# NREL/SSRS

Hardware: AMD Instinct MI355X
Metric: simulated tracks/sec (whole node) (higher is better)
Workload: dtype f64

## Files before the change

ssrs_amd/csrc/tracks.hip:

```cpp
#include <rocrand/rocrand_philox4x32_10.h>
#include <hipcub/hipcub.hpp>

#include <cmath>
#include <cstdlib>
#include <cstring>
#include <new>
#include <vector>

#include "common.h"
#include "track_plan.h"
#include "track_policy.h"

namespace ssrs {

__host__ __device__ constexpr int dr_of(int k) { return k / 3 - 1; }
__host__ __device__ constexpr int dc_of(int k) { return k % 3 - 1; }
#define SSRS_NINV_DIAG 0.70710677f

constexpr uint32_t restriction(int d)
{
    const int dr = dr_of(d), dc = dc_of(d);
    uint32_t m = 0;
    for (int k = 0; k < 9; ++k) {
        bool ok = false;
        if (dr == 0 && dc == 0) ok = true;
        else if (dr != 0 && dc != 0)
            ok = (dr_of(k) == dr || dr_of(k) == 0) && (dc_of(k) == dc || dc_of(k) == 0);
        else if (dr == 0) ok = dc_of(k) == dc;
        else ok = dr_of(k) == dr;
        if (ok && k != 4) m |= 1u << k;
    }
    return m;
}
constexpr uint64_t pack_restrictions(int first, int count)
{
    uint64_t v = 0;
    for (int i = 0; i < count; ++i) v |= static_cast<uint64_t>(restriction(first + i)) << (9 * i);
    return v;
}
constexpr uint64_t kRestrictLo = pack_restrictions(0, 7);
constexpr uint64_t kRestrictHi = pack_restrictions(7, 2);
constexpr uint32_t kAllButCentre = restriction(4);
static_assert(restriction(0) == 0b000001011u, "(-1,-1) -> k in {0,1,3}");
static_assert(restriction(7) == 0b111000000u, "(1,0) -> k in {6,7,8}");
static_assert(kAllButCentre == 0b111101111u, "(0,0) -> all but centre");

__device__ __forceinline__ uint32_t restriction_of(uint32_t d)
{
    const uint64_t v = d < 7 ? (kRestrictLo >> (9 * d)) : (kRestrictHi >> (9 * (d - 7)));
    return static_cast<uint32_t>(v) & 0x1FFu;
}

constexpr uint32_t candidates(int d)
{
    uint32_t v = 0;
    int n = 0;
    for (int k = 0; k < 9 && n < 3; ++k)
        if ((restriction(d) >> k) & 1u) v |= static_cast<uint32_t>(k < 4 ? k : k - 1) << (3 * n++);
    return v;
}
constexpr uint64_t pack_candidates(int first, int count)
{
    uint64_t v = 0;
    for (int i = 0; i < count; ++i) v |= static_cast<uint64_t>(candidates(first + i)) << (9 * i);
    return v;
}
constexpr uint64_t kCandLo = pack_candidates(0, 7), kCandHi = pack_candidates(7, 2);
static_assert(candidates(7) == (5u | (6u << 3) | (7u << 6)), "(1,0) -> table slots 5,6,7");
static_assert(candidates(5) == (2u | (4u << 3) | (7u << 6)), "(0,1) -> k = 2,5,8 = slots 2,4,7");

__device__ __forceinline__ uint32_t candidates_of(uint32_t d)
{
    const uint64_t v = d < 7 ? (kCandLo >> (9 * d)) : (kCandHi >> (9 * (d - 7)));
    return static_cast<uint32_t>(v) & 0x1FFu;
}

constexpr int kRingK[8] = {7, 8, 5, 2, 1, 0, 3, 6};
constexpr int ring_of_k(int k)
{
    for (int c = 0; c < 8; ++c)
        if (kRingK[c] == k) return c;
    return 8;
}
constexpr bool ring_matches_restrictions()
{
    for (int c = 0; c < 8; ++c) {
        const uint32_t m = (1u << kRingK[(c + 7) % 8]) | (1u << kRingK[c]) | (1u << kRingK[(c + 1) % 8]);
        if (m != restriction(kRingK[c])) return false;
    }
// ... 478 lines not shown
template <typename KeyT>
__global__ __launch_bounds__(kBlock) void k_plan_keys(const int32_t *__restrict__ start_rc,
                                                     long long ntracks, PlanGeom g,
                                                     KeyT *__restrict__ keys,
                                                     int32_t *__restrict__ vals, TrackCtl *ctl, int par_bits)
{
    const long long t = blockIdx.x * static_cast<long long>(kBlock) + threadIdx.x;
    int par = 0x7fffffff;
    if (t < ntracks) {
        int perp;
        plan_coords(g, start_rc[2 * t], start_rc[2 * t + 1], par, perp);
        par = par < 0 ? 0 : par;
        perp = perp < 0 ? 0 : perp;
        const int top = (1 << par_bits) - 1;
        keys[t] = (static_cast<KeyT>(perp > top ? top : perp) << par_bits) | static_cast<KeyT>(par > top ? top : par);
        vals[t] = static_cast<int32_t>(t);
    }
    __shared__ int s_min;
    if (threadIdx.x == 0) s_min = 0x7fffffff;
    __syncthreads();
#pragma unroll
    for (int off = 32; off > 0; off >>= 1) {
        const int o = __shfl_down(par, off);
        par = o < par ? o : par;
    }
    if ((threadIdx.x & 63) == 0 && par != 0x7fffffff) atomicMin(&s_min, par);
    __syncthreads();
    if (threadIdx.x == 0 && s_min != 0x7fffffff) atomicMin(&ctl->par_min, static_cast<uint32_t>(s_min));
}

__device__ __forceinline__ int wander_window_of(const WanderWindows *__restrict__ w, int n, int row, int col)
{
    int id = n;
    for (int q = n - 1; q >= 0; --q)
        if (static_cast<uint32_t>(row - w->r0[q]) < static_cast<uint32_t>(kWinRows) &&
            static_cast<uint32_t>(col - w->c0[q]) < static_cast<uint32_t>(kWinCols)) id = q;
    return id;
}

enum { MODE_PRIOR = 0, MODE_UPDRAFT = 1, MODE_FLUIDFLOW = 2, MODE_TABLE = 3 };

struct RoamEntry;

struct StepArgs {
    int rows, cols, burnin, memory;
    long long max_k;
    double nu;
    const double *prior;
    const double *updraft;
    const float *potential;
    const double *table;
    unsigned long long seed, track_base;
    uint32_t *hist;
    int16_t *end_rc;
    int32_t *lengths;
    int16_t *traj;
    const long long *traj_off;
    TrackState *state;
    const int32_t *list_in;
    int32_t *list_out;
    TrackCtl *ctl;
    int launch;
    int fast;
    int steps;
    int coherent;
    uint32_t *visits;
    long long visit_stride;
    uint32_t cap;
    long long it_base;
    int plane_shift;
    uint32_t guard;
    int v16_offset;
    int pf_dir, pf_rc;
    uint32_t vcap;
    const double *thr;
    const uint8_t *zmask;
    uint32_t *hist_copies;
    int ncopies;
    const WanderWindows *wander;
    const RoamEntry *roam;
    const void *fine;
    int roam_stop;
    int cheap_exact;
    unsigned long long *dbg_buf;
    int debug_roam;
    uint32_t vis_r, vis_c;
};

__global__ __launch_bounds__(kBlock) void k_tracks_init(
    const int32_t *__restrict__ start_rc, long long ntracks, int rows, int cols,
    uint32_t *hist, int16_t *traj, const long long *traj_off, int32_t *lengths,
    int16_t *end_rc, TrackState *state, TrackCtl *ctl, PlanGeom g, int coherent, uint32_t cap)
{
    const long long t = blockIdx.x * static_cast<long long>(kBlock) + threadIdx.x;
    if (t < kXcd) {
        const long long left = ntracks - t * static_cast<long long>(cap);
        ctl->count[0][t] = static_cast<uint32_t>(left < 0 ? 0 : (left > cap ? cap : left));
        ctl->count[1][t] = ctl->count[2][t] = ctl->count[3][t] = 0;
        if (t == 0) ctl->steps = 0;
    }
    if (t >= ntracks) return;
    const int row = start_rc[2 * t], col = start_rc[2 * t + 1];
    TrackState s;
    s.dirs = 0x44444444u;
    uint32_t delay = 0;
    if (coherent) {
        int par, perp;
        plan_coords(g, row, col, par, perp);
        par = par < 0 ? 0 : par;
        const uint32_t pmin = ctl->par_min;
        delay = static_cast<uint32_t>(par) > pmin ? static_cast<uint32_t>(par) - pmin : 0u;
        if (delay > 0x7FFFFFu) delay = 0x7FFFFFu;
        delay &= ~1u;
    }
    s.aux = kAllButCentre | (delay << 9);
    if (row < 0 || col < 0 || row >= rows || col >= cols) {
        atomicOr(&ctl->error, 1u);
        s.pos = 0;
        s.k = -1;
        if (lengths) lengths[t] = 0;
        if (end_rc) { end_rc[2 * t] = -1; end_rc[2 * t + 1] = -1; }
    } else {
        s.pos = row | (col << 16);
        s.k = 0;
        if (hist) atomicAdd(&hist[static_cast<size_t>(row) * cols + col], 1u);
        if (traj)
            reinterpret_cast<uint32_t *>(traj)[traj_off[t]] =
                static_cast<uint32_t>(row & 0xFFFF) | (static_cast<uint32_t>(col) << 16);
    }
    state[t] = s;
}

template <int MODE>
__global__ __launch_bounds__(kBlock) void k_step_tracks(const StepArgs a)
{
    TrackCtl *ctl = a.ctl;
    const int in_slot = a.launch & 3, out_slot = (a.launch + 1) & 3;
    const uint32_t xcd = blockIdx.x % kXcd;
    const uint32_t nlive = ctl->count[in_slot][xcd];
    const uint32_t il = (blockIdx.x / kXcd) * kBlock + threadIdx.x;
    const uint32_t i = xcd * a.cap + il;
    const uint32_t iv = xcd * a.vcap + il;
    if (blockIdx.x == 0 && threadIdx.x < kXcd)
        ctl->count[(a.launch + 2) & 3][threadIdx.x] = 0;
    if ((il & ~63u) >= nlive) return;

    bool active = il < nlive;
    const int32_t t = active ? (a.list_in ? a.list_in[i] : static_cast<int32_t>(i)) : 0;
    TrackState s = {0, -1, 0, 0};
    if (active) s = a.state[t];
    active = active && s.k >= 0;
    int row = s.pos & 0xFFFF, col = (s.pos >> 16) & 0xFFFF;
    int k = s.k;
    const int max_k = static_cast<int>(a.max_k);
    uint32_t dirs = s.dirs, run = s.aux & 0x1FFu;
    const long long rel64 = (a.coherent ? static_cast<long long>(s.aux >> 9) : 0) -
                            static_cast<long long>(a.launch) * a.steps;
    const int release = rel64 > 0x7fffffffLL ? 0x7fffffff : (rel64 < 0 ? 0 : static_cast<int>(rel64));
    const unsigned long long track = a.track_base + static_cast<unsigned long long>(t);
    const long long toff = (a.traj && active) ? a.traj_off[t] : 0;
    const long long troom = (a.traj && active) ? a.traj_off[t + 1] - toff : 0;
    uint32_t pend_a = 0, pend_b = 0;
    bool have_pending = false;
    uint32_t moved = 0;
    int last_it = -1;

// ... 1072 lines not shown
struct FineEntry { uint32_t t1, t2; };
struct FinePrior { uint32_t zero_t1[8], zero_t2[8], reversal; };

__host__ __device__ __forceinline__ uint32_t fine_fixed(double x)
{
    const double v = x * 4294967296.0 + 0.5;
    return v >= 4294967295.0 ? 0xFFFFFFFFu : static_cast<uint32_t>(static_cast<unsigned long long>(v));
}

template <bool HAS_POT>
__global__ __launch_bounds__(kBlock) void k_fine_build(const double *__restrict__ updraft, const float *__restrict__ potential,
                                                      FineEntry *__restrict__ out, int rows, int cols, int tiles_x, int ntiles,
                                                      const FinePrior fp)
{
    constexpr int LW = kTabW + 2, LH = kTabH + 2;
    __shared__ double s_inv[LW * LH];
    __shared__ float s_pot[LW * LH];
    const int t = xcd_band(blockIdx.x, ntiles);
    const int r0 = (t / tiles_x) * kTabH, c0 = (t % tiles_x) * kTabW;
    for (int i = threadIdx.x; i < LW * LH; i += kBlock) {
        const int lr = i / LW, lc = i - lr * LW;
        int gr = r0 - 1 + lr, gc = c0 - 1 + lc;
        gr = gr < 0 ? 0 : (gr >= rows ? rows - 1 : gr);
        gc = gc < 0 ? 0 : (gc >= cols ? cols - 1 : gc);
        const size_t g = static_cast<size_t>(gr) * cols + gc;
        const double v = updraft[g];
        const double w = v != v ? v : (v > 1e-06 ? v : 1e-06);
        s_inv[i] = 1.0 / w;
        s_pot[i] = HAS_POT ? potential[g] : 0.f;
    }
    __syncthreads();
    const int lc = static_cast<int>(threadIdx.x % kTabW) + 1;
    const int col = c0 + lc - 1;
    if (col >= cols) return;
    for (int lr = static_cast<int>(threadIdx.x / kTabW) + 1; lr <= kTabH; lr += kBlock / kTabW) {
        const int row = r0 + lr - 1;
        if (row >= rows) break;
        const size_t cell = static_cast<size_t>(row) * cols + col;
        const bool interior = row > 0 && col > 0 && row < rows - 1 && col < cols - 1;
        double w[9];
        bool bad = !interior;
        if (interior) {
            const double ic = s_inv[lr * LW + lc];
            const float pc = s_pot[lr * LW + lc];
#pragma unroll
            for (int j = 0; j < 9; ++j) {
                const int o = (lr + dr_of(j)) * LW + lc + dc_of(j);
                w[j] = 2.0 / (ic + s_inv[o]);
                if (HAS_POT) {
                    const float d = pc - s_pot[o];
                    const float ninv = (j == 4) ? 0.f : ((j & 1) ? 1.f : SSRS_NINV_DIAG);
                    const float e = d * ninv;
                    w[j] = w[j] * static_cast<double>(e);
                }
                bad |= !(w[j] - w[j] == 0.0);
                w[j] = w[j] > 0.0 ? w[j] : 0.0;
            }
        }
        FineEntry en[8];
#pragma unroll
        for (int rc = 0; rc < 8; ++rc) {
            const uint32_t ord = ring_order(rc);
            const int ring3[3] = {(rc + 7) % 8, rc, (rc + 1) % 8};
            const int ka = kRingK[ring3[ord & 3u]], kb = kRingK[ring3[(ord >> 2) & 3u]], kc = kRingK[ring3[(ord >> 4) & 3u]];
            FineEntry e = {0xFFFFFFFFu, 0u};
            if (!bad) {
                const double ab = w[ka] + w[kb], tot = ab + w[kc];
                if (tot == 0.0) {
                    if (!((fp.reversal >> rc) & 1u)) { e.t1 = fp.zero_t1[rc]; e.t2 = fp.zero_t2[rc]; }
                } else if (tot - tot == 0.0) {
                    e.t1 = fine_fixed(w[ka] / tot);
                    e.t2 = fine_fixed(ab / tot);
                    if (e.t1 > e.t2) e.t1 = e.t2;
                }
            }
            en[rc] = e;
        }
        uint4 *dst = reinterpret_cast<uint4 *>(out + cell * 8);
#pragma unroll
        for (int q = 0; q < 4; ++q) dst[q] = make_uint4(en[2 * q].t1, en[2 * q].t2, en[2 * q + 1].t1, en[2 * q + 1].t2);
    }
}

template <bool REV, int BT = kBlock>
__global__ __launch_bounds__(BT) void k_step_roam(const StepArgs a, const ThrPrior pr)
{
    __shared__ uint32_t s_win[kWinRows * kWinCols];
    __shared__ int s_box[4];
    __shared__ int s_wid[BT / 64];
    for (int q = threadIdx.x; q < kWinRows * kWinCols; q += BT) s_win[q] = 0u;
    if (threadIdx.x == 0) { s_box[0] = s_box[1] = 0x7fffffff; s_box[2] = s_box[3] = -1; }
    __syncthreads();
    TrackCtl *ctl = a.ctl;
    const int in_slot = a.launch & 3, out_slot = (a.launch + 1) & 3;
    const uint32_t xcd = blockIdx.x % kXcd;
    const uint32_t nlive = ctl->count[in_slot][xcd];
    const uint32_t il = (blockIdx.x / kXcd) * BT + threadIdx.x;
    const uint32_t i = xcd * a.cap + il;
    if (blockIdx.x == 0 && threadIdx.x < kXcd) ctl->count[(a.launch + 2) & 3][threadIdx.x] = 0;

    bool live0 = il < nlive;
    int32_t t = live0 ? (a.list_in ? a.list_in[i] : static_cast<int32_t>(i)) : 0;
    if (t < 0) { live0 = false; t = 0; }
    TrackState s = {0, -1, 0, 0};
    if (live0) s = a.state[t];
    uint32_t rc = static_cast<uint32_t>(kRingOfK >> (4 * (s.dirs & 0xFu))) & 0xFu;
    live0 = live0 && s.k >= 0 && rc < 8u;
    rc &= 7u;
    int row = s.pos & 0xFFFF, col = (s.pos >> 16) & 0xFFFF;
    int win_r0 = 0, win_c0 = 0;
    {
        int r_lo = live0 ? row : 0x7fffffff, r_hi = live0 ? row : -1, c_lo = live0 ? col : 0x7fffffff, c_hi = live0 ? col : -1;
#pragma unroll
        for (int off = 32; off > 0; off >>= 1) {
            int o = __shfl_xor(r_lo, off); r_lo = o < r_lo ? o : r_lo;
            o = __shfl_xor(r_hi, off); r_hi = o > r_hi ? o : r_hi;
            o = __shfl_xor(c_lo, off); c_lo = o < c_lo ? o : c_lo;
            o = __shfl_xor(c_hi, off); c_hi = o > c_hi ? o : c_hi;
        }
        if ((threadIdx.x & 63) == 0 && r_hi >= 0) {
            atomicMin(&s_box[0], r_lo); atomicMin(&s_box[1], c_lo);
            atomicMax(&s_box[2], r_hi); atomicMax(&s_box[3], c_hi);
        }
        __syncthreads();
        const bool fits = s_box[2] - s_box[0] < kWinRows && s_box[3] - s_box[1] < kWinCols;
        const int nwin = a.wander->n;
        int wid = live0 && nwin > 0 ? wander_window_of(a.wander, nwin, row, col) : 0x7fffffff;
        wid = wid >= nwin ? 0x7fffffff : wid;
        {
            const unsigned long long lm = __ballot(wid != 0x7fffffff);
            wid = lm ? __shfl(wid, __ffsll(static_cast<long long>(lm)) - 1) : 0x7fffffff;
        }
        if ((threadIdx.x & 63) == 0) s_wid[threadIdx.x >> 6] = wid;
        __syncthreads();
        wid = 0x7fffffff;
        for (int q = BT / 64 - 1; q >= 0; --q) wid = s_wid[q] != 0x7fffffff ? s_wid[q] : wid;
        if (wid != 0x7fffffff && threadIdx.x == 0) {
            s_box[0] = a.wander->r0[wid]; s_box[2] = s_box[0] + kWinRows - 1;
            s_box[1] = a.wander->c0[wid]; s_box[3] = s_box[1] + kWinCols - 1;
        }
        const bool placed = wid != 0x7fffffff;
        __syncthreads();
        if (!placed && !fits && threadIdx.x == 0) { s_box[0] = r_lo; s_box[1] = c_lo; s_box[2] = r_hi; s_box[3] = c_hi; }
        __syncthreads();
        if (s_box[2] >= 0) {
            win_r0 = (s_box[0] + s_box[2] + 1 - kWinRows) / 2;
            win_c0 = (s_box[1] + s_box[3] + 1 - kWinCols) / 2;
        }
    }
    const char *pair = reinterpret_cast<const char *>(a.roam);
    const uint32_t ucols = static_cast<uint32_t>(a.cols);
    const uint32_t last_cell = static_cast<uint32_t>(a.rows) * ucols - 1u;
    int k = s.k;
    const long long rel64 = (a.coherent ? static_cast<long long>(s.aux >> 9) : 0) + 1 - a.it_base;
    const int rel = rel64 > 0x3fffffffLL ? 0x3fffffff : (rel64 < 0 ? 0 : static_cast<int>(rel64));
    const long long left = a.max_k - k;
    uint32_t span = !live0 ? 0u : (left > 0x3fffffffLL ? 0x3fffffffu : (left < 0 ? 0u : static_cast<uint32_t>(left)));
    const int blk0 = (k - rel) >> 1;
    const unsigned long long track = a.track_base + static_cast<unsigned long long>(t);
    const char *tab = reinterpret_cast<const char *>(a.table);
    const uint32_t psh = static_cast<uint32_t>(a.plane_shift);
    const uint32_t rev_e = pr.rev_e;
    uint32_t win_stray = 0, n_fine = 0;
    const void *fine = a.fine;

    int wr = 0, wc = 0, lcell = 0;
// ... 9 lines not shown
    };
    enter(rel == 0);
    const uint32_t rev_rc4 = 4u * pr.rev_rc;

    auto slow_step = [&](const uint32_t w0, const uint32_t w1) __attribute__((always_inline)) {
        const uint32_t ufi = w0 >> 16;
        const uint32_t cell = static_cast<uint32_t>(row) * ucols + static_cast<uint32_t>(col);
        const uint32_t e = *reinterpret_cast<const uint32_t *>(tab + (a.guard + (rc << psh)) + (cell << 2));
        const int32_t d1 = static_cast<int32_t>(ufi) - static_cast<int32_t>(e & 0xFFFFu);
        const int32_t d2 = static_cast<int32_t>(ufi) - static_cast<int32_t>(e >> 16);
        const bool burn = k <= a.burnin;
        bool special = (static_cast<uint32_t>(d1 + 1) < 2u) | (static_cast<uint32_t>(d2 + 1) < 2u) | (d1 < d2);
        if (burn) special |= (row <= 1) | (row >= a.rows - 2) | (col >= a.cols - 2);
        uint32_t nc;
        int br = row, bc = col;
        if (!special) {
            const uint32_t ord = static_cast<uint32_t>(kRingOrder >> (6u * rc)) & 63u;
            const uint32_t neg = (static_cast<uint32_t>(d1) >> 31) + (static_cast<uint32_t>(d2) >> 31);
            nc = (rc + 7u + ((ord >> (4u - 2u * neg)) & 3u)) & 7u;
        } else {
            if (e == kThrBoundary && !burn) { span = 0u; return; }
            bool exact = true;
            nc = 0;
            if (fine && !(d1 < d2) && !(burn && ((row <= 1) | (row >= a.rows - 2) | (col >= a.cols - 2)))) {
                const uint2 f = reinterpret_cast<const uint2 *>(fine)[(cell << 3) | rc];
                const uint32_t u32 = (w0 & ~31u) | (w1 >> 27);
                const long long f1 = static_cast<long long>(u32) - static_cast<long long>(f.x);
                const long long f2 = static_cast<long long>(u32) - static_cast<long long>(f.y);
                const bool unsure = (f.x > f.y) | (static_cast<unsigned long long>(f1 + 1) < 2ull) | (static_cast<unsigned long long>(f2 + 1) < 2ull);
                if (!unsure) {
                    const uint32_t ord = static_cast<uint32_t>(kRingOrder >> (6u * rc)) & 63u;
                    const uint32_t neg = (f1 < 0 ? 1u : 0u) + (f2 < 0 ? 1u : 0u);
                    nc = (rc + 7u + ((ord >> (4u - 2u * neg)) & 3u)) & 7u;
                    exact = false;
                    ++n_fine;
                }
            }
            if (e == kThrReversal && !burn) {
                int idx = 0;
                bool near = false;
#pragma unroll
                for (int q = 0; q < 9; ++q) {
                    const int32_t d = static_cast<int32_t>(ufi) - static_cast<int32_t>(pr.thr9[q]);
                    idx += d >= 0 ? 1 : 0;
                    near |= static_cast<uint32_t>(d + 1) < 2u;
                }
                const uint32_t pnc = static_cast<uint32_t>(kRingOfK >> (4 * (idx > 8 ? 4 : idx))) & 0xFu;
                if (!near && pnc < 8u) { nc = pnc; exact = false; }
            }
            if (exact) {
                int er = row, ec = col;
                if (burn) {
                    if (er <= 1) er += 2; else if (er >= a.rows - 2) er -= 2;
                    if (ec <= 0) ec += 2; else if (ec >= a.cols - 2) ec -= 2;
                }
                double w[9];
                if (a.potential) window_weights<true>(a.updraft, a.potential, a.cols, er, ec, w);
                else window_weights<false>(a.updraft, a.potential, a.cols, er, ec, w);
                double prr[9];
#pragma unroll
                for (int j = 0; j < 9; ++j) prr[j] = a.prior[j];
                const uint32_t last = static_cast<uint32_t>(kKOfRing >> (4 * rc)) & 0xFu;
                const int idx = choose_move(w, prr, 1.0, restriction_of(last), words_to_uniform(w0, w1), true);
                nc = static_cast<uint32_t>(kRingOfK >> (4 * idx)) & 0xFu;
                br = er; bc = ec;
            }
        }
        row = br + static_cast<int>((kRingDr >> (2u * nc)) & 3u) - 1;
        col = bc + static_cast<int>((kRingDc >> (2u * nc)) & 3u) - 1;
        rc = nc;
        ++k;
        const uint32_t hr = static_cast<uint32_t>(row - win_r0), hc = static_cast<uint32_t>(col - win_c0);
        if (hr < static_cast<uint32_t>(kWinRows) && hc < static_cast<uint32_t>(kWinCols)) {
            atomicAdd(&s_win[hr * kWinCols + hc], 1u);
        } else {
            atomicAdd(&a.hist[static_cast<uint32_t>(row) * ucols + static_cast<uint32_t>(col)], 1u);
            ++win_stray;
        }
    };

    int it = 0;
    uint32_t n_pairs = 0, n_slow = 0;
    const unsigned long long t_begin = a.debug_roam ? __builtin_amdgcn_s_memtime() : 0ull;
    auto one_pair = [&]() __attribute__((always_inline)) {
        const uint4 w4 = philox_block_b3(a.seed, track, static_cast<unsigned long long>(static_cast<uint32_t>(blk0 + (it >> 1))));
        const uint32_t ufa = w4.x >> 16, ufb = w4.z >> 16;
        const bool st_a = static_cast<uint32_t>(it - rel) < span, st_b = static_cast<uint32_t>(it + 1 - rel) < span;
        const uint32_t q0 = E.x, qa = E.y, qb = E.z, qc = E.w;
        const uint32_t rc0 = rc;
        const uint32_t rc04 = 4u * rc0;
        const bool rva = REV && q0 == kThrReversal;
        const uint32_t eua = rva ? rev_e : q0;
        const uint32_t t4a = rva ? rev_rc4 : rc04;
        const bool ga1 = ufa >= (eua & 0xFFFFu), ga2 = ufa >= (eua >> 16);
        const uint32_t nxa = ga2 ? kRingNext2 : (ga1 ? kRingNext1 : kRingNext0);
        const uint32_t nca = (nxa >> t4a) & 7u, nca4 = 4u * nca;
        const uint32_t q1 = ga2 ? qc : (ga1 ? qb : qa);
        const int dra = __builtin_amdgcn_sbfe(static_cast<int>(kRingDrS), nca4, 2u), dca = __builtin_amdgcn_sbfe(static_cast<int>(kRingDcS), nca4, 2u);
        const int cell_a = lcell + __mul24(dra, a.cols) + dca;
        const bool rvb = REV && q1 == kThrReversal;
        const uint32_t eub = rvb ? rev_e : q1;
        const uint32_t t4b = rvb ? rev_rc4 : nca4;
        const bool gb1 = ufb >= (eub & 0xFFFFu), gb2 = ufb >= (eub >> 16);
        const uint32_t nxb = gb2 ? kRingNext2 : (gb1 ? kRingNext1 : kRingNext0);
        const uint32_t ncb = (nxb >> t4b) & 7u, ncb4 = 4u * ncb;
        const int drb = __builtin_amdgcn_sbfe(static_cast<int>(kRingDrS), ncb4, 2u), dcb = __builtin_amdgcn_sbfe(static_cast<int>(kRingDcS), ncb4, 2u);
        const int cell_b = cell_a + __mul24(drb, a.cols) + dcb;
        {
            const uint32_t cb = static_cast<uint32_t>(cell_b) < last_cell ? static_cast<uint32_t>(cell_b) : last_cell;
            E = *reinterpret_cast<const uint4 *>(pair + ((cb << 7) | (ncb4 << 2)));
        }
        const int wra = wr + dra, wca = wc + dca, wrb = wra + drb, wcb = wca + dcb;
        const int32_t a1 = static_cast<int32_t>(ufa) - static_cast<int32_t>(eua & 0xFFFFu);
        const int32_t a2 = static_cast<int32_t>(ufa) - static_cast<int32_t>(eua >> 16);
        const int32_t b1 = static_cast<int32_t>(ufb) - static_cast<int32_t>(eub & 0xFFFFu);
        const int32_t b2 = static_cast<int32_t>(ufb) - static_cast<int32_t>(eub >> 16);
        const bool special = (static_cast<uint32_t>(a1 + 1) < 2u) | (static_cast<uint32_t>(a2 + 1) < 2u) | (a1 < a2) |
                             (static_cast<uint32_t>(b1 + 1) < 2u) | (static_cast<uint32_t>(b2 + 1) < 2u) | (b1 < b2);
        const bool go = fast & st_a & st_b & !special;
        const bool in_a = go & (static_cast<uint32_t>(wra) < static_cast<uint32_t>(kWinRows)) & (static_cast<uint32_t>(wca) < static_cast<uint32_t>(kWinCols));
        const bool in_b = go & (static_cast<uint32_t>(wrb) < static_cast<uint32_t>(kWinRows)) & (static_cast<uint32_t>(wcb) < static_cast<uint32_t>(kWinCols));
        const bool out = go & !(in_a & in_b);
        const bool slow = (st_a | st_b) & !go;
        const unsigned long long rare = __ballot(out | slow);
        atomicAdd(&s_win[in_a ? (wra << 8) + wca : 0], in_a ? 1u : 0u);
        atomicAdd(&s_win[in_b ? (wrb << 8) + wcb : 0], in_b ? 1u : 0u);
        k += go ? 2 : 0;
        wr = go ? wrb : wr;
        wc = go ? wcb : wc;
        lcell = go ? cell_b : lcell;
        rc = go ? ncb : rc0;
        ++n_pairs;
        if (__builtin_expect(rare != 0ull, 0)) {
            if (__any(out)) {
#ifdef SSRS_PROBE_NO_STRAY_ATOMICS
                if (go && !in_a) ++win_stray;
                if (go && !in_b) ++win_stray;
#else
                if (go && !in_a) { atomicAdd(&a.hist[cell_a], 1u); ++win_stray; }
                if (go && !in_b) { atomicAdd(&a.hist[cell_b], 1u); ++win_stray; }
#endif
            }
            if (__any(slow)) {
                ++n_slow;
                if (slow) {
                    if (fast) { row = win_r0 + wr; col = win_c0 + wc; }
#pragma unroll 1
                    for (int h = 0; h < 2; ++h)
                        if (static_cast<uint32_t>(it + h - rel) < span) slow_step(h ? w4.z : w4.x, h ? w4.w : w4.y);
                    enter(true);
                }
            }
        }
        it += 2;
    };
    const uint32_t stop_stamp = static_cast<uint32_t>(a.launch) + 1u;
    uint32_t stop_seen = 0u;
    bool stopped = false;
    for (; it + 8 <= a.steps; ) {
        const unsigned long long stepping = __ballot(static_cast<uint32_t>(it - rel) < span), waiting = __ballot(it < rel && span != 0u);
        const bool stop_now = a.roam_stop && waiting == 0ull &&
                              static_cast<uint32_t>(__builtin_amdgcn_readfirstlane(static_cast<int>(stop_seen))) == stop_stamp;
        if (((stepping | waiting) == 0ull) | stop_now) { stopped = stop_now; break; }
        if (a.roam_stop) stop_seen = __hip_atomic_load(&ctl->roam_stop, __ATOMIC_RELAXED, __HIP_MEMORY_SCOPE_AGENT);
#pragma unroll
        for (int u = 0; u < 4; ++u) one_pair();
    }
    for (; it < a.steps && !stopped; ) {
        if (!__any(static_cast<uint32_t>(it - rel) < span || (it < rel && span != 0u))) break;
        one_pair();
    }
    if (a.roam_stop && !stopped && it >= a.steps && (threadIdx.x & 63) == 0) atomicMax(&ctl->roam_stop, stop_stamp);
    if (fast) { row = win_r0 + wr; col = win_c0 + wc; }
    {
        uint32_t nf = n_fine;
#pragma unroll
        for (int off = 32; off > 0; off >>= 1) nf += __shfl_down(nf, off);
        if ((threadIdx.x & 63) == 0 && nf) atomicAdd(&ctl->pad, nf);
    }
    if ((threadIdx.x & 63) == 0 && n_pairs) {
        atomicAdd(&ctl->roam_pairs, static_cast<unsigned long long>(n_pairs));
        if (n_slow) atomicAdd(&ctl->roam_slow, static_cast<unsigned long long>(n_slow));
        if (a.debug_roam) {
            const unsigned long long dt = __builtin_amdgcn_s_memtime() - t_begin;
            atomicAdd(&ctl->dbg_tsum, dt);
            atomicMax(&ctl->dbg_tmax, dt);
            atomicAdd(&ctl->dbg_waves, 1ull);
            atomicMax(&ctl->dbg_slowmax, (static_cast<unsigned long long>(n_slow) << 32) | n_pairs);
        }
    }
#ifdef SSRS_DEBUG_WAVE_DUMP
    if (a.debug_roam && a.launch == SSRS_DEBUG_WAVE_DUMP && a.dbg_buf) {
        const unsigned long long dt = __builtin_amdgcn_s_memtime() - t_begin;
        const int lanes = __popcll(__ballot(live0));
        uint32_t wst = win_stray;
        for (int off = 32; off > 0; off >>= 1) wst += __shfl_down(wst, off);
        if ((threadIdx.x & 63) == 0) {
            unsigned long long *r = a.dbg_buf + 8ull * (blockIdx.x * (BT / 64) + (threadIdx.x >> 6));
            r[0] = dt; r[1] = static_cast<unsigned long long>(lanes); r[2] = n_pairs; r[3] = n_slow; r[4] = wst;
            r[5] = static_cast<unsigned long long>(win_r0); r[6] = static_cast<unsigned long long>(win_c0);
            r[7] = static_cast<uint32_t>(__popcll(__ballot(fast)));
        }
    }
#endif
    __syncthreads();
    for (int q = threadIdx.x; q < kWinRows * kWinCols; q += BT) {
        const uint32_t n = s_win[q];
        if (n) atomicAdd(&a.hist[static_cast<uint32_t>(win_r0 + q / kWinCols) * ucols + static_cast<uint32_t>(win_c0 + q % kWinCols)], n);
    }
    {
        unsigned long long ws = win_stray;
#pragma unroll
        for (int off = 32; off > 0; off >>= 1) ws += __shfl_down(ws, off);
        if ((threadIdx.x & 63) == 0 && ws) atomicAdd(&ctl->strays, ws);
    }
    const bool active = live0 && span != 0u && k < static_cast<int>(a.max_k);
    if (live0 && !active) {
        if (a.lengths) a.lengths[t] = static_cast<int32_t>(k + 1);
        if (a.end_rc) reinterpret_cast<uint32_t *>(a.end_rc)[t] = (static_cast<uint32_t>(row) & 0xFFFFu) | (static_cast<uint32_t>(col) << 16);
    }
    __shared__ uint32_t s_surv[BT / 64 + 1];
    const int lane = threadIdx.x & 63, wv = threadIdx.x >> 6;
    const int nsurv = __popcll(__ballot(active));
    if (lane == 0) s_surv[wv] = static_cast<uint32_t>(nsurv);
    __syncthreads();
    if (threadIdx.x == 0) {
        uint32_t tot = 0;
        for (int q = 0; q < BT / 64; ++q) tot += s_surv[q];
        s_surv[BT / 64] = tot ? atomicAdd(&ctl->count[out_slot][xcd], static_cast<uint32_t>(BT)) : 0xFFFFFFFFu;
    }
    __syncthreads();
    const uint32_t basei = s_surv[BT / 64];
    if (basei != 0xFFFFFFFFu) {
        a.list_out[xcd * a.cap + basei + threadIdx.x] = active ? t : -1;
        if (active) {
            TrackState o;
            o.pos = static_cast<int32_t>((static_cast<uint32_t>(row) & 0xFFFFu) | (static_cast<uint32_t>(col) << 16));
            o.k = k;
            o.dirs = static_cast<uint32_t>(kKOfRing >> (4 * rc)) & 0xFu;
            o.aux = s.aux;
            a.state[t] = o;
        }
    }
    unsigned long long mv = live0 ? static_cast<unsigned long long>(k - s.k) : 0ull;
#pragma unroll
    for (int off = 32; off > 0; off >>= 1) mv += __shfl_down(mv, off);
    if (lane == 0 && mv) atomicAdd(&ctl->steps, mv);
}

constexpr int kBinThreads = 1024;
constexpr int kBinCells = 30720;
__global__ __launch_bounds__(kBinThreads) void k_bin_visits(const uint32_t *__restrict__ visits,
                                                           long long stride,
// ... 871 lines not shown
    return SSRS_OK;
}

extern "C" size_t ssrs_transition_ring_bytes(int rows, int cols)
{
    if (rows <= 0 || cols <= 0) return 0;
    const size_t cells = static_cast<size_t>(rows) * static_cast<size_t>(cols);
    return ring_mask_offset(rows, cols) + (cells + 3) / 4 * 4;
}

extern "C" int ssrs_transition_ring_build(const double *updraft, const float *potential,
                                          float *ring, int rows, int cols, void *stream)
{
    SSRS_REQUIRE(updraft && ring, "ssrs_transition_ring_build: updraft/ring is NULL");
    SSRS_REQUIRE(rows >= 3 && cols >= 3, "ssrs_transition_ring_build: need rows, cols >= 3");
    SSRS_REQUIRE((reinterpret_cast<uintptr_t>(ring) & 7u) == 0,
                 "ssrs_transition_ring_build: ring must be 8-byte aligned");
    const int tx = (cols + kTabW - 1) / kTabW, ty = (rows + kTabH - 1) / kTabH, nt = tx * ty;
    hipLaunchKernelGGL(k_transition_table<true>, dim3(static_cast<unsigned>(nt)), dim3(kBlock), 0,
                       as_stream(stream), updraft, potential, static_cast<void *>(ring), rows, cols, tx, nt);
    SSRS_HIP_CHECK(hipGetLastError());
    return SSRS_OK;
}

static size_t thr_guard_bytes(int cols) { return align_up((static_cast<size_t>(cols) + 2) * 4, 256); }

extern "C" size_t ssrs_transition_thr_bytes(int rows, int cols)
{
    if (rows <= 0 || cols <= 0) return 0;
    return (static_cast<size_t>(8) << thr_plane_shift(rows, cols)) + 2 * thr_guard_bytes(cols);
}

extern "C" int ssrs_transition_thr_build(const double *updraft, const float *potential,
                                         const double *prior, float *thr, int rows, int cols, void *stream)
{
    SSRS_REQUIRE(updraft && thr && prior, "ssrs_transition_thr_build: updraft/prior/thr is NULL");
    SSRS_REQUIRE(rows >= 3 && cols >= 3, "ssrs_transition_thr_build: need rows, cols >= 3");
    SSRS_REQUIRE(static_cast<size_t>(rows) * static_cast<size_t>(cols) <= (1ull << 26),
                 "ssrs_transition_thr_build: the table and its guard bands are addressed with 32-bit offsets (rows * cols <= 2^26)");
    SSRS_REQUIRE((reinterpret_cast<uintptr_t>(thr) & 63u) == 0,
                 "ssrs_transition_thr_build: table must be 64-byte aligned");
    ThrPrior pr;
    prior_tables(prior, &pr);
    const int tx = (cols + kTabW - 1) / kTabW, ty = (rows + kTabH - 1) / kTabH, nt = tx * ty;
    uint32_t *planes = reinterpret_cast<uint32_t *>(reinterpret_cast<char *>(thr) + thr_guard_bytes(cols));
    ThrHeader *header = reinterpret_cast<ThrHeader *>(thr);
    PriorArg heading;
    for (int k = 0; k < 9; ++k) heading.v[k] = prior[k];
    if (potential)
        hipLaunchKernelGGL(k_transition_thr<true>, dim3(static_cast<unsigned>(nt)), dim3(kBlock), 0, as_stream(stream),
                           updraft, potential, planes, rows, cols, tx, nt, pr, thr_plane_shift(rows, cols), header, heading);
    else
        hipLaunchKernelGGL(k_transition_thr<false>, dim3(static_cast<unsigned>(nt)), dim3(kBlock), 0, as_stream(stream),
                           updraft, potential, planes, rows, cols, tx, nt, pr, thr_plane_shift(rows, cols), header, heading);
    SSRS_HIP_CHECK(hipGetLastError());
    return SSRS_OK;
}

extern "C" int ssrs_uniform_selftest(uint64_t seed, const uint64_t *track, const uint64_t *step,
                                     double *out, size_t n, void *stream)
{
    SSRS_REQUIRE(track && step && out, "ssrs_uniform_selftest: NULL pointer");
    if (n == 0) return SSRS_OK;
    hipLaunchKernelGGL(k_uniform_selftest, dim3(static_cast<unsigned>((n + 255) / 256)), dim3(256),
                       0, as_stream(stream), seed, track, step, out, n);
    SSRS_HIP_CHECK(hipGetLastError());
    return SSRS_OK;
}


struct TrackCall {
    const SsrsTrackParams *p;
    const double *updraft; const float *potential; const double *table;
    const int32_t *start_rc; int64_t ntracks; uint64_t seed, track_id_base;
    uint32_t *hist; int16_t *end_rc; int32_t *lengths; int16_t *traj; const int64_t *traj_offsets;
    void *workspace; size_t workspace_bytes; void *stream;
    SsrsTrajRecorder *rec;
    unsigned long long *hist64;
};

struct TrackSwitches {
    bool debug, debug_roam;
    bool roam_stop, cheap_exact, block_window, fine_table, roam_table, rev, deal_contiguous, rebalance, grow_steps;
    long long roam_wide_from;
    int roam_width;
    int roam_shuffle;
};

static TrackSwitches read_track_switches()
{
    auto set = [](const char *name) { return std::getenv(name) != nullptr; };
    TrackSwitches sw;
    sw.debug = set("SSRS_TRACKS_DEBUG");
    sw.debug_roam = set("SSRS_TRACKS_DEBUG_ROAM");
    sw.roam_stop = !set("SSRS_TRACKS_NO_ROAM_STOP");
    sw.cheap_exact = !set("SSRS_TRACKS_NO_CHEAP_EXACT");
    sw.block_window = !set("SSRS_TRACKS_NO_BLOCK_WINDOW");
    sw.fine_table = !set("SSRS_TRACKS_NO_FINE_TABLE");
    sw.roam_table = !set("SSRS_TRACKS_NO_ROAM_TABLE");
    sw.rev = !set("SSRS_TRACKS_NO_REV");
    sw.deal_contiguous = !set("SSRS_TRACKS_DEAL_ROUND_ROBIN");
    sw.rebalance = !set("SSRS_TRACKS_NO_REBALANCE");
    sw.grow_steps = !set("SSRS_TRACKS_FIXED_STEPS");
    sw.roam_wide_from = static_cast<long long>(kDealBlocks + kWanderWindows - 2) * kBlock + 1;
    if (const char *e = std::getenv("SSRS_TRACKS_ROAM_WIDE")) sw.roam_wide_from = std::atoll(e);
    sw.roam_width = 0;
    if (const char *e = std::getenv("SSRS_TRACKS_ROAM_WIDTH")) { const int w = std::atoi(e); if (w == 1 || w == 2 || w == 4) sw.roam_width = w; }
    sw.roam_shuffle = 16;
    if (const char *e = std::getenv("SSRS_TRACKS_ROAM_SHUFFLE")) sw.roam_shuffle = std::atoi(e);
    return sw;
}

static_assert(offsetof(TrackCtl, steps) == kSlotSteps * sizeof(uint32_t) &&
              offsetof(TrackCtl, strays) == kSlotSteps * sizeof(uint32_t) + sizeof(unsigned long long), "read-back slot");

struct TrackEvents {
    hipEvent_t first = nullptr, last = nullptr;
    hipEvent_t batch[kRing] = {};
    bool own_batch = false;
    std::vector<hipEvent_t> marks;
    std::vector<int> kind;
    TrackEvents() = default;
    TrackEvents(const TrackEvents &) = delete;
    TrackEvents &operator=(const TrackEvents &) = delete;
    ~TrackEvents()
    {
        for (hipEvent_t e : marks) (void)hipEventDestroy(e);
        if (own_batch)
            for (hipEvent_t e : batch)
                if (e) (void)hipEventDestroy(e);
        if (first) (void)hipEventDestroy(first);
        if (last) (void)hipEventDestroy(last);
    }
};

static int check_track_args(const TrackCall &c)
{
    const SsrsTrackParams *p = c.p;
    SSRS_REQUIRE(p != nullptr, "ssrs_tracks_simulate: params is NULL");
    SSRS_REQUIRE(c.hist64 == nullptr || c.hist != nullptr, "ssrs_tracks_simulate_h64: the 32-bit raster the kernels count into is NULL");
    SSRS_REQUIRE(p->rows >= 5 && p->cols >= 5, "ssrs_tracks_simulate: need rows, cols >= 5 (got %d x %d)",
                 p->rows, p->cols);
    SSRS_REQUIRE(p->rows <= 32767 && p->cols <= 32767,
                 "ssrs_tracks_simulate: rows, cols must fit int16 trajectories (<= 32767)");
    SSRS_REQUIRE(p->memory_parameter >= 0 && p->memory_parameter <= 8,
                 "ssrs_tracks_simulate: memory_parameter must be in 0..8 (got %d)",
                 p->memory_parameter);
    SSRS_REQUIRE(p->max_moves >= 0 && p->max_moves < (1ll << 31) - 1,
                 "ssrs_tracks_simulate: max_moves out of range");
    SSRS_REQUIRE(p->burnin >= 0, "ssrs_tracks_simulate: burnin must be >= 0");
    SSRS_REQUIRE(c.ntracks >= 0 && c.ntracks < (1ll << 31) - 64, "ssrs_tracks_simulate: bad ntracks");
    SSRS_REQUIRE(!(c.potential && !c.updraft && !c.table),
                 "ssrs_tracks_simulate: potential_field needs updraft_field (reference raises)");
    SSRS_REQUIRE(!(c.traj && !c.traj_offsets), "ssrs_tracks_simulate: traj needs traj_offsets");
    SSRS_REQUIRE(!(c.table && (reinterpret_cast<uintptr_t>(c.table) & 63u)),
                 "ssrs_tracks_simulate: table must be 64-byte aligned");
    return SSRS_OK;
}

struct TrackRun {
    const TrackCall c;
    const SsrsTrackParams *p;
    const TrackSwitches sw;
    hipStream_t st;
    Workspace ws = {};
    uint32_t *host_counts = nullptr;
    int S = 0, mode = 0, mode0 = 0;
    bool profile = false, coherent = false, lean = false, ring = false, thr = false;
    PlanGeom geom = {};
    ThrPrior thr_prior = {};
    StepArgs a = {};
    uint32_t ntc = 0, ntiles = 0;
    size_t ncell = 0;
    bool roam_ok = false, rev = false, wander_sort_ok = false, v16_ok = false;
    uint32_t *hist_t = nullptr;
    uint32_t *copies_ptr = nullptr;
    int ncopies = 0;
    bool copies_live = false;
    unsigned long long private_visits = 0;
    bool roam_ready = false;
    int roam_width = 1;
    TrackPolicy pol;
    int launch = 0, batches = 0, last_Sl = 0;
    long long it_done = 0;
    int window_launches = 0, tile_launches = 0, block_window_launches = 0, roam_launches = 0, roam_wide_launches = 0;
    int slot_row[kRing] = {};
// ... 42 lines not shown
    if (bad)
        return set_error(SSRS_ERR_INVALID, "ssrs_tracks_simulate: `table` is not a threshold table built by "
                         "ssrs_transition_thr_build for this %d x %d raster and params->prior (nothing was launched)",
                         p->rows, p->cols);
    return SSRS_OK;
}

int TrackRun::plan_and_init()
{
    const int64_t ntracks = c.ntracks;
    SSRS_HIP_CHECK(hipEventCreate(&ev.first));
    SSRS_HIP_CHECK(hipEventCreate(&ev.last));
    SSRS_HIP_CHECK(hipEventRecord(ev.first, st));
    {
        PriorArg pa;
        for (int k = 0; k < 9; ++k) pa.v[k] = p->prior[k];
        const ThrHeader *header = (p->flags & SSRS_TRACKS_THR_TABLE) ? reinterpret_cast<const ThrHeader *>(c.table) : nullptr;
        hipLaunchKernelGGL(k_ctl_init, dim3(1), dim3(64), 0, st, ws.ctl, pa, ws.thr, ws.wander, header, p->rows, p->cols);
        SSRS_HIP_CHECK(hipGetLastError());
    }
    coherent = (p->flags & SSRS_TRACKS_NO_SCHEDULE) == 0;
    const unsigned blocks = static_cast<unsigned>((ntracks + kBlock - 1) / kBlock);
    if (coherent) {
        double vr = 0.0, vc = 0.0;
        for (int k = 0; k < 9; ++k) { vr += p->prior[k] * dr_of(k); vc += p->prior[k] * dc_of(k); }
        const double nrm = std::sqrt(vr * vr + vc * vc);
        geom.cos_t = nrm > 0.0 ? vr / nrm : 1.0;
        geom.sin_t = nrm > 0.0 ? vc / nrm : 0.0;
        geom.offset = p->rows + p->cols;
        int par_bits = 1;
        while ((1ll << par_bits) <= 2ll * geom.offset) ++par_bits;
        size_t temp_bytes = ws.sort_temp_bytes;
        if (2 * par_bits <= 32) {
            uint32_t *k0 = reinterpret_cast<uint32_t *>(ws.keys[0]), *k1 = reinterpret_cast<uint32_t *>(ws.keys[1]);
            hipLaunchKernelGGL(k_plan_keys<uint32_t>, dim3(blocks), dim3(kBlock), 0, st, c.start_rc,
                               static_cast<long long>(ntracks), geom, k0, ws.list[1], ws.ctl, par_bits);
            SSRS_HIP_CHECK(hipGetLastError());
            SSRS_HIP_CHECK(hipcub::DeviceRadixSort::SortPairs(
                ws.sort_temp, temp_bytes, k0, k1, ws.list[1], ws.list[0], static_cast<int>(ntracks), 0, 2 * par_bits, st));
        } else {
            hipLaunchKernelGGL(k_plan_keys<unsigned long long>, dim3(blocks), dim3(kBlock), 0, st, c.start_rc,
                               static_cast<long long>(ntracks), geom, ws.keys[0], ws.list[1], ws.ctl, par_bits);
            SSRS_HIP_CHECK(hipGetLastError());
            SSRS_HIP_CHECK(hipcub::DeviceRadixSort::SortPairs(
                ws.sort_temp, temp_bytes, ws.keys[0], ws.keys[1], ws.list[1], ws.list[0],
                static_cast<int>(ntracks), 0, 2 * par_bits, st));
        }
    }
    hipLaunchKernelGGL(k_tracks_init, dim3(blocks), dim3(kBlock), 0, st, c.start_rc,
                       static_cast<long long>(ntracks), p->rows, p->cols, c.hist, c.traj,
                       reinterpret_cast<const long long *>(c.traj_offsets), c.lengths, c.end_rc,
                       ws.state, ws.ctl, geom, coherent ? 1 : 0, ws.cap);
    SSRS_HIP_CHECK(hipGetLastError());

    S = p->steps_per_launch > 0 ? p->steps_per_launch : 512;
    profile = (p->flags & SSRS_TRACKS_PROFILE) != 0;
    mode = c.table ? MODE_TABLE : (c.updraft ? (c.potential ? MODE_FLUIDFLOW : MODE_UPDRAFT) : MODE_PRIOR);
    mode0 = c.updraft ? (c.potential ? MODE_FLUIDFLOW : MODE_UPDRAFT) : MODE_PRIOR;
    a.rows = p->rows; a.cols = p->cols; a.burnin = p->burnin; a.memory = p->memory_parameter;
    a.max_k = p->max_moves; a.nu = p->scaling_parameter;
    a.prior = ws.ctl->prior;
    a.updraft = c.updraft; a.potential = c.potential; a.table = c.table;
    a.seed = c.seed; a.track_base = c.track_id_base;
    a.hist = c.hist; a.end_rc = c.end_rc; a.lengths = c.lengths; a.traj = c.traj;
    a.traj_off = reinterpret_cast<const long long *>(c.traj_offsets);
    a.state = ws.state; a.ctl = ws.ctl; a.steps = S;
    a.fast = ((p->flags & SSRS_TRACKS_EXACT_ONLY) == 0 && p->scaling_parameter == 1.0) ? 1 : 0;
    a.coherent = coherent ? 1 : 0;
    a.cap = ws.cap;
    a.thr = ws.thr;
    a.wander = ws.wander;
    a.debug_roam = sw.debug_roam ? 1 : 0;
    a.roam_stop = sw.roam_stop ? 1 : 0;
    a.dbg_buf = nullptr;
#ifdef SSRS_DEBUG_WAVE_DUMP
    {
        static unsigned long long *dump_buf = nullptr;
        if (!dump_buf && a.debug_roam && hipMalloc(&dump_buf, 8ull * 8 * 4096 * (kBlock / 64)) != hipSuccess) dump_buf = nullptr;
        if (dump_buf) (void)hipMemsetAsync(dump_buf, 0, 8ull * 8 * 4096 * (kBlock / 64), st);
        a.dbg_buf = dump_buf;
    }
#endif
    a.cheap_exact = sw.cheap_exact ? 1 : 0;
    a.vcap = ws.cap;
    lean = p->memory_parameter == 1 && c.traj == nullptr;
    ring = (p->flags & SSRS_TRACKS_RING_TABLE) != 0;
    thr = (p->flags & SSRS_TRACKS_THR_TABLE) != 0;
    if (thr) {
        SSRS_REQUIRE(!ring && c.table && c.updraft && lean && a.fast && (S & 1) == 0,
                     "ssrs_tracks_simulate: SSRS_TRACKS_THR_TABLE needs table + updraft, memory_parameter 1, "
                     "scaling_parameter 1, no direct trajectory output, no EXACT_ONLY and an even steps_per_launch");
        SSRS_REQUIRE(static_cast<size_t>(p->rows) * static_cast<size_t>(p->cols) <= (1ull << 26),
                     "ssrs_tracks_simulate: the threshold table needs rows * cols <= 2^26");
        prior_tables(p->prior, &thr_prior);
        a.plane_shift = thr_plane_shift(p->rows, p->cols);
        a.guard = static_cast<uint32_t>(thr_guard_bytes(p->cols));
        a.pf_dir = coherent ? (geom.cos_t > 0.98 ? 1 : (geom.cos_t < -0.98 ? -1 : 0)) : 0;
        a.pf_rc = a.pf_dir < 0 ? 4 : 0;
    }
    if (ring)
        SSRS_REQUIRE(c.table && c.updraft && lean && a.fast && (S & 1) == 0,
                     "ssrs_tracks_simulate: SSRS_TRACKS_RING_TABLE needs table + updraft, memory_parameter 1, "
                     "scaling_parameter 1, no trajectory output, no EXACT_ONLY and an even steps_per_launch");
    return SSRS_OK;
}

int TrackRun::choose_front_path()
{
    const int64_t ntracks = c.ntracks;
    uint32_t *const hist = c.hist;
    const double off_axis = std::fabs(geom.sin_t) < std::fabs(geom.cos_t) ? std::fabs(geom.sin_t) : std::fabs(geom.cos_t);
    ntc = static_cast<uint32_t>((p->cols + kTileCols - 1) / kTileCols);
    ntiles = ntc * static_cast<uint32_t>((p->rows + kTileRows - 1) / kTileRows);
    const bool tiles_ok = hist != nullptr && coherent && S <= kVisitSteps && ntracks >= 8192 && ntiles <= kTilesMax &&
                          static_cast<unsigned long long>(ws.cap) * kXcd * static_cast<unsigned long long>(S) < (1ull << 32) &&
                          (p->flags & SSRS_TRACKS_NO_BINNING) == 0;
    bool tiles_on = tiles_ok && off_axis > 0.17;
    const bool want_transposed = coherent && !tiles_on && std::fabs(geom.sin_t) > std::fabs(geom.cos_t);
    const bool binning = hist != nullptr && coherent && S <= kVisitSteps &&
                         (p->flags & SSRS_TRACKS_NO_BINNING) == 0 &&
                         (want_transposed ? p->rows : p->cols) <= kBinCells;
    a.visits = nullptr;
    a.visit_stride = ws.visit_stride;
    bool binning_on = binning && ntracks >= 8192 && !tiles_on;
    const bool never_scattered = (p->flags & SSRS_TRACKS_NO_SCATTERED) != 0;
    const bool scattered = (p->flags & SSRS_TRACKS_SCATTERED) != 0;
    if (scattered) binning_on = tiles_on = false;
    const bool cache_ok = thr && hist != nullptr && !(c.rec && c.rec->complete) && sw.block_window;
    size_t ws_base = align_up(ssrs_tracks_workspace_bytes(ntracks), 256);
    {
        const size_t pb = thr ? pair_table_bytes(ntracks, p->rows, p->cols) : 0;
        if (pb && c.workspace_bytes >= ws_base + pb) {
            ws.roam = reinterpret_cast<RoamEntry *>(static_cast<char *>(c.workspace) + ws_base);
            if (sw.fine_table)
                a.fine = static_cast<char *>(c.workspace) + ws_base +
                         align_up(static_cast<size_t>(p->rows) * static_cast<size_t>(p->cols) * 8 * sizeof(RoamEntry), 256);
            ws_base += pb;
        }
        a.roam = ws.roam;
    }
    roam_ok = cache_ok && ws.roam != nullptr && sw.roam_table;
    rev = thr_prior.rev_ok != 0 && sw.rev;
    wander_sort_ok = ntracks >= kWanderMinTracks &&
                     static_cast<long long>((p->rows + kBinRows - 1) / kBinRows) * ((p->cols + kBinCols - 1) / kBinCols) <= kWanderBins;
    ncell = static_cast<size_t>(p->rows) * static_cast<size_t>(p->cols);
    if (hist && c.workspace_bytes > ws_base) ncopies = static_cast<int>((c.workspace_bytes - ws_base) / (ncell * sizeof(uint32_t)));
    uint32_t *extra = reinterpret_cast<uint32_t *>(static_cast<char *>(c.workspace) + ws_base);
    if (want_transposed && binning_on) {
        if (ncopies >= 1) { hist_t = extra; extra += ncell; --ncopies; }
        else binning_on = false;
    }
    if (hist_t) SSRS_HIP_CHECK(hipMemsetAsync(hist_t, 0, sizeof(uint32_t) * ncell, st));
    ncopies = ncopies > 64 ? 64 : ncopies;
    copies_ptr = ncopies >= 2 ? extra : nullptr;
    a.hist_copies = nullptr;
    a.ncopies = 1;
    a.zmask = ring ? reinterpret_cast<const uint8_t *>(c.table) + ring_mask_offset(p->rows, p->cols) : nullptr;
    v16_ok = 5ll * p->cols <= kBinCells;
    a.v16_offset = geom.offset;

    pol.thr = thr; pol.tiles_ok = tiles_ok; pol.cache_ok = cache_ok; pol.never_scattered = never_scattered;
    pol.front = a.pf_dir != 0; pol.may_rebalance = sw.rebalance; pol.debug = sw.debug; pol.roam_shuffle = sw.roam_shuffle;
    pol.ntracks = ntracks; pol.crossing = p->rows + p->cols;
    pol.binning_on = binning_on; pol.tiles_on = tiles_on; pol.scattered = scattered;
    pol.cached = cache_ok && scattered;
    pol.want_wander_sort = pol.cached;
// ... 568 lines not shown
```

Before: 74580.

## Add steady-state roam loop specializations with lane-mask predication

The roaming step loop now classifies each 8-step trip. When every stepping lane is fast and stays in span for the whole trip, it runs specialized versions of the pair step that drop the per-step span checks and use a precomputed wave mask, converted to a per-lane flag with inverse_ballot. A masked variant also skips the whole trip body for inactive lanes and guards the shared-memory atomics with branches instead of dummy adds. This adds code size, register pressure and more control flow, and the roam-stop flag is read mid-trip from the first active lane.

```diff
diff --git a/ssrs_amd/csrc/tracks.hip b/ssrs_amd/csrc/tracks.hip
--- a/ssrs_amd/csrc/tracks.hip
+++ b/ssrs_amd/csrc/tracks.hip
@@ -5,6 +5,7 @@
 #include <cstdlib>
 #include <cstring>
 #include <new>
+#include <type_traits>
 #include <vector>
 
 #include "common.h"
@@ -649,6 +650,8 @@
     const void *fine;
     int roam_stop;
     int cheap_exact;
+    int roam_steady;
+    int roam_mask;
     unsigned long long *dbg_buf;
     int debug_roam;
     uint32_t vis_r, vis_c;
@@ -1887,6 +1890,11 @@
     }
 }
 
+__device__ __forceinline__ bool lane_of_mask(unsigned long long mask)
+{
+    return __builtin_amdgcn_inverse_ballot_w64(mask);
+}
+
 template <bool REV, int BT = kBlock>
 __global__ __launch_bounds__(BT) void k_step_roam(const StepArgs a, const ThrPrior pr)
 {
@@ -2062,10 +2070,11 @@
     int it = 0;
     uint32_t n_pairs = 0, n_slow = 0;
     const unsigned long long t_begin = a.debug_roam ? __builtin_amdgcn_s_memtime() : 0ull;
-    auto one_pair = [&]() __attribute__((always_inline)) {
-        const uint4 w4 = philox_block_b3(a.seed, track, static_cast<unsigned long long>(static_cast<uint32_t>(blk0 + (it >> 1))));
+    auto one_pair = [&](auto steady_c, auto mask_c, const int itp, unsigned long long &on) __attribute__((always_inline)) -> bool {
+        constexpr bool STEADY = decltype(steady_c)::value, MASK = decltype(mask_c)::value;
+        const uint4 w4 = philox_block_b3(a.seed, track, static_cast<unsigned long long>(static_cast<uint32_t>(blk0 + (itp >> 1))));
         const uint32_t ufa = w4.x >> 16, ufb = w4.z >> 16;
-        const bool st_a = static_cast<uint32_t>(it - rel) < span, st_b = static_cast<uint32_t>(it + 1 - rel) < span;
+        const bool st_a = STEADY || static_cast<uint32_t>(itp - rel) < span, st_b = STEADY || static_cast<uint32_t>(itp + 1 - rel) < span;
         const uint32_t q0 = E.x, qa = E.y, qb = E.z, qc = E.w;
         const uint32_t rc0 = rc;
         const uint32_t rc04 = 4u * rc0;
@@ -2097,20 +2106,26 @@
         const int32_t b2 = static_cast<int32_t>(ufb) - static_cast<int32_t>(eub >> 16);
         const bool special = (static_cast<uint32_t>(a1 + 1) < 2u) | (static_cast<uint32_t>(a2 + 1) < 2u) | (a1 < a2) |
                              (static_cast<uint32_t>(b1 + 1) < 2u) | (static_cast<uint32_t>(b2 + 1) < 2u) | (b1 < b2);
-        const bool go = fast & st_a & st_b & !special;
+        const bool lane_on = STEADY ? lane_of_mask(on) : false;
+        const bool go = STEADY ? (lane_on & !special) : (fast & st_a & st_b & !special);
         const bool in_a = go & (static_cast<uint32_t>(wra) < static_cast<uint32_t>(kWinRows)) & (static_cast<uint32_t>(wca) < static_cast<uint32_t>(kWinCols));
         const bool in_b = go & (static_cast<uint32_t>(wrb) < static_cast<uint32_t>(kWinRows)) & (static_cast<uint32_t>(wcb) < static_cast<uint32_t>(kWinCols));
         const bool out = go & !(in_a & in_b);
-        const bool slow = (st_a | st_b) & !go;
+        const bool slow = STEADY ? (lane_on & special) : ((st_a | st_b) & !go);
         const unsigned long long rare = __ballot(out | slow);
-        atomicAdd(&s_win[in_a ? (wra << 8) + wca : 0], in_a ? 1u : 0u);
-        atomicAdd(&s_win[in_b ? (wrb << 8) + wcb : 0], in_b ? 1u : 0u);
+        if constexpr (MASK) {
+            if (in_a) atomicAdd(&s_win[(wra << 8) + wca], 1u);
+            if (in_b) atomicAdd(&s_win[(wrb << 8) + wcb], 1u);
+        } else {
+            atomicAdd(&s_win[in_a ? (wra << 8) + wca : 0], in_a ? 1u : 0u);
+            atomicAdd(&s_win[in_b ? (wrb << 8) + wcb : 0], in_b ? 1u : 0u);
+        }
         k += go ? 2 : 0;
         wr = go ? wrb : wr;
         wc = go ? wcb : wc;
         lcell = go ? cell_b : lcell;
         rc = go ? ncb : rc0;
-        ++n_pairs;
+        bool any_slow = false;
         if (__builtin_expect(rare != 0ull, 0)) {
             if (__any(out)) {
 #ifdef SSRS_PROBE_NO_STRAY_ATOMICS
@@ -2122,33 +2137,79 @@
 #endif
             }
             if (__any(slow)) {
-                ++n_slow;
+                any_slow = true;
                 if (slow) {
                     if (fast) { row = win_r0 + wr; col = win_c0 + wc; }
 #pragma unroll 1
                     for (int h = 0; h < 2; ++h)
-                        if (static_cast<uint32_t>(it + h - rel) < span) slow_step(h ? w4.z : w4.x, h ? w4.w : w4.y);
+                        if (static_cast<uint32_t>(itp + h - rel) < span) slow_step(h ? w4.z : w4.x, h ? w4.w : w4.y);
                     enter(true);
                 }
+                if constexpr (STEADY) on &= __ballot(fast);
             }
         }
-        it += 2;
+        return any_slow;
     };
+    const std::true_type yes;
+    const std::false_type no;
+    unsigned long long on = 0ull;
     const uint32_t stop_stamp = static_cast<uint32_t>(a.launch) + 1u;
     uint32_t stop_seen = 0u;
     bool stopped = false;
-    for (; it + 8 <= a.steps; ) {
-        const unsigned long long stepping = __ballot(static_cast<uint32_t>(it - rel) < span), waiting = __ballot(it < rel && span != 0u);
-        const bool stop_now = a.roam_stop && waiting == 0ull &&
-                              static_cast<uint32_t>(__builtin_amdgcn_readfirstlane(static_cast<int>(stop_seen))) == stop_stamp;
-        if (((stepping | waiting) == 0ull) | stop_now) { stopped = stop_now; break; }
+    enum { kTripDone = 0, kTripGeneric, kTripSteady, kTripMasked };
+    bool lane_on = false;
+    int first_on = 0;
+    auto next_trip = [&](const uint32_t flag) __attribute__((always_inline)) -> int {
+        if (it + 8 > a.steps) return kTripDone;
+        const bool lane_steps = static_cast<uint32_t>(it - rel) < span;
+        const unsigned long long stepping = __ballot(lane_steps), waiting = __ballot(it < rel && span != 0u);
+        const bool stop_now = a.roam_stop && waiting == 0ull && flag == stop_stamp;
+        if (((stepping | waiting) == 0ull) | stop_now) { stopped = stop_now; return kTripDone; }
         if (a.roam_stop) stop_seen = __hip_atomic_load(&ctl->roam_stop, __ATOMIC_RELAXED, __HIP_MEMORY_SCOPE_AGENT);
-#pragma unroll
-        for (int u = 0; u < 4; ++u) one_pair();
-    }
-    for (; it < a.steps && !stopped; ) {
+        lane_on = fast & lane_steps & (static_cast<uint32_t>(it + 7 - rel) < span);
+        on = __ballot(lane_on);
+        first_on = __ffsll(static_cast<long long>(on)) - 1;
+        if (!(a.roam_steady && on == stepping && waiting == 0ull)) return kTripGeneric;
+        return a.roam_mask ? kTripMasked : kTripSteady;
+    };
+    auto generic_trip = [&]() __attribute__((always_inline)) {
+#pragma unroll
+        for (int u = 0; u < 4; ++u) n_slow += one_pair(no, no, it + 2 * u, on) ? 1u : 0u;
+        n_pairs += 4;
+        it += 8;
+    };
+    auto flag_seen = [&]() __attribute__((always_inline)) { return static_cast<uint32_t>(__builtin_amdgcn_readfirstlane(static_cast<int>(stop_seen))); };
+    int kind = next_trip(flag_seen());
+    while (kind == kTripGeneric) { generic_trip(); kind = next_trip(flag_seen()); }
+    if (kind == kTripMasked) {
+        do {
+            unsigned long long on_t = on;
+            uint32_t trip_slow = 0, seen = 0;
+            if (lane_on) {
+                trip_slow += one_pair(yes, yes, it, on_t) ? 1u : 0u;
+                seen = flag_seen();
+#pragma unroll
+                for (int u = 1; u < 4; ++u) trip_slow += one_pair(yes, yes, it + 2 * u, on_t) ? 1u : 0u;
+            }
+            n_slow += static_cast<uint32_t>(__builtin_amdgcn_readlane(static_cast<int>(trip_slow), first_on));
+            n_pairs += 4;
+            it += 8;
+            kind = next_trip(static_cast<uint32_t>(__builtin_amdgcn_readlane(static_cast<int>(seen), first_on)));
+        } while (kind == kTripMasked);
+    } else if (kind == kTripSteady) {
+        do {
+            unsigned long long on_t = on;
+#pragma unroll
+            for (int u = 0; u < 4; ++u) n_slow += one_pair(yes, no, it + 2 * u, on_t) ? 1u : 0u;
+            n_pairs += 4;
+            it += 8;
+        } while ((kind = next_trip(flag_seen())) == kTripSteady);
+    }
+    while (kind != kTripDone) { generic_trip(); kind = next_trip(flag_seen()); }
+    for (; it < a.steps && !stopped; it += 2) {
         if (!__any(static_cast<uint32_t>(it - rel) < span || (it < rel && span != 0u))) break;
-        one_pair();
+        n_slow += one_pair(no, no, it, on) ? 1u : 0u;
+        ++n_pairs;
     }
     if (a.roam_stop && !stopped && it >= a.steps && (threadIdx.x & 63) == 0) atomicMax(&ctl->roam_stop, stop_stamp);
     if (fast) { row = win_r0 + wr; col = win_c0 + wc; }
@@ -3186,6 +3247,7 @@
 struct TrackSwitches {
     bool debug, debug_roam;
     bool roam_stop, cheap_exact, block_window, fine_table, roam_table, rev, deal_contiguous, rebalance, grow_steps;
+    bool roam_steady, roam_mask;
     long long roam_wide_from;
     int roam_width;
     int roam_shuffle;
@@ -3206,6 +3268,8 @@
     sw.deal_contiguous = !set("SSRS_TRACKS_DEAL_ROUND_ROBIN");
     sw.rebalance = !set("SSRS_TRACKS_NO_REBALANCE");
     sw.grow_steps = !set("SSRS_TRACKS_FIXED_STEPS");
+    sw.roam_steady = !set("SSRS_TRACKS_NO_ROAM_STEADY");
+    sw.roam_mask = !set("SSRS_TRACKS_ROAM_LOAD_ALL");
     sw.roam_wide_from = static_cast<long long>(kDealBlocks + kWanderWindows - 2) * kBlock + 1;
     if (const char *e = std::getenv("SSRS_TRACKS_ROAM_WIDE")) sw.roam_wide_from = std::atoll(e);
     sw.roam_width = 0;
@@ -3414,6 +3478,8 @@
     }
 #endif
     a.cheap_exact = sw.cheap_exact ? 1 : 0;
+    a.roam_steady = sw.roam_steady ? 1 : 0;
+    a.roam_mask = sw.roam_mask ? 1 : 0;
     a.vcap = ws.cap;
     lean = p->memory_parameter == 1 && c.traj == nullptr;
     ring = (p->flags & SSRS_TRACKS_RING_TABLE) != 0;
```

After: 70600. -5.3%, worse.
